# ThatRedox/ChunkyClPlugin

Hardware: NVIDIA B200
Metric: path samples/sec (higher is better)
Workload: dtype f32

## Files before the change

### chunkyclplugin_b200/csrc/ccu_layout.h

```cpp
#pragma once
#include <algorithm>
#include <cmath>
#include <cstdint>
#include <cstdlib>
#include <cstring>
#include <thread>
#include <unordered_map>
#include <vector>

#include "ccu_device.cuh"
#include "ccu_march.cuh"

namespace {
struct WideLayout {
    std::vector<unsigned> top, wide;
    int cell_level = 0, top_log2 = 0;
    bool ok = true;
};

inline unsigned wide_leaf(int word, int level, bool &ok) {
    long long v = -(long long)word;
    unsigned val;
    if (v == 0x7FFFFFFELL) val = CCU_WIDE_ANY;
    else if (v >= 0 && v < (long long)CCU_WIDE_ANY) val = (unsigned)v;
    else { ok = false; val = 0; }
    return CCU_WIDE_LEAF | ((unsigned)level << 26) | val;
}

unsigned wide_node(const int *tree, size_t n, int word, int lvl, WideLayout &b) {
    if (lvl < 2 || (size_t)word + 7 >= n) { b.ok = false; return wide_leaf(0, 0, b.ok); }
    const size_t idx = b.wide.size() / 64;
    if (idx >= 0x7FFFFFFFu) { b.ok = false; return wide_leaf(0, 0, b.ok); }
    b.wide.resize(b.wide.size() + 64);
    for (int i = 0; i < 4; i++)
        for (int j = 0; j < 4; j++)
            for (int k = 0; k < 4; k++) {
                unsigned e;
                int c1 = tree[(size_t)word + ((((i >> 1) & 1) << 2) | (((j >> 1) & 1) << 1) | ((k >> 1) & 1))];
                if (c1 <= 0) {
                    e = wide_leaf(c1, lvl - 1, b.ok);
                } else if ((size_t)c1 + 7 >= n) {
                    b.ok = false;
                    e = wide_leaf(0, 0, b.ok);
                } else {
                    int c2 = tree[(size_t)c1 + (((i & 1) << 2) | ((j & 1) << 1) | (k & 1))];
                    e = c2 <= 0 ? wide_leaf(c2, lvl - 2, b.ok) : wide_node(tree, n, c2, lvl - 2, b);
                }
                b.wide[idx * 64 + ((i << 4) | (j << 2) | k)] = e;
            }
    return (unsigned)idx;
}

struct AirLayout {
    std::vector<unsigned> top, wide, bricks;
    std::vector<unsigned char> wide_level;
    int cell_level = 4, top_log2 = 0;
    bool ok = true;
};

inline int layout_threads(int dim) {
    if (dim < 8) return 1;
    if (const char *e = getenv("CCU_COMMIT_THREADS")) return std::max(1, std::min(dim, atoi(e)));
    const unsigned hw = std::thread::hardware_concurrency();
    return (int)std::max(1u, std::min({hw ? hw : 4u, (unsigned)dim, 16u}));
}

inline unsigned air_leaf(int word, int level) { return CCU_WIDE_LEAF | ((word == 0 ? (unsigned)level : 31u) << 26); }
inline int oct_child(int x, int y, int z) { return ((x & 1) << 2) | ((y & 1) << 1) | (z & 1); }

unsigned air_brick(const int *tree, size_t n, int word, AirLayout &b) {
    const size_t idx = b.bricks.size() / 256;
    if (idx >= 0x7FFFFFu || (size_t)word + 7 >= n) { b.ok = false; return air_leaf(1, 0); }
    b.bricks.resize(b.bricks.size() + 256, 0u);
    for (int i = 0; i < 4; i++)
        for (int j = 0; j < 4; j++)
            for (int k = 0; k < 4; k++) {
                unsigned *blk = &b.bricks[idx * 256 + (size_t)((i << 4) | (j << 2) | k) * 4];
                unsigned uniform = 0;
                bool mixed = false;
                int c2 = 0;
                const int c1 = tree[(size_t)word + oct_child(i >> 1, j >> 1, k >> 1)];
                if (c1 <= 0) {
                    uniform = c1 == 0 ? (CCU_BRICK_UNIFORM | 3u) : 0u;
                } else if ((size_t)c1 + 7 >= n) {
                    b.ok = false;
                } else {
                    c2 = tree[(size_t)c1 + oct_child(i, j, k)];
                    if (c2 <= 0) uniform = c2 == 0 ? (CCU_BRICK_UNIFORM | 2u) : 0u;
                    else if ((size_t)c2 + 7 >= n) b.ok = false;
                    else mixed = true;
                }
                if (!mixed) {
                    blk[0] = blk[1] = blk[2] = blk[3] = uniform;
                    continue;
                }
                for (int x = 0; x < 4; x++)
                    for (int y = 0; y < 4; y++)
                        for (int z = 0; z < 4; z++) {
                            unsigned code;
                            const int d1 = tree[(size_t)c2 + oct_child(x >> 1, y >> 1, z >> 1)];
                            if (d1 <= 0) {
                                code = d1 == 0 ? 2u : 0u;
                            } else if ((size_t)d1 + 7 >= n) {
                                b.ok = false;
                                code = 0;
                            } else {
                                const int d2 = tree[(size_t)d1 + oct_child(x, y, z)];
                                if (d2 > 0) b.ok = false;
                                code = d2 == 0 ? 1u : 0u;
                            }
                            blk[x] |= code << ((((y << 2) | z)) * 2);
                        }
            }
    return (unsigned)idx;
}

unsigned air_node(const int *tree, size_t n, int word, int lvl, AirLayout &b) {
    if (lvl == 4) return air_brick(tree, n, word, b);
    if (lvl < 6 || (size_t)word + 7 >= n) { b.ok = false; return air_leaf(1, 0); }
    const size_t idx = b.wide.size() / 64;
    if (idx >= 0x1FFFFFFu) { b.ok = false; return air_leaf(1, 0); }
    b.wide.resize(b.wide.size() + 64);
    b.wide_level.push_back((unsigned char)lvl);
    for (int i = 0; i < 4; i++)
        for (int j = 0; j < 4; j++)
            for (int k = 0; k < 4; k++) {
                unsigned e;
                const int c1 = tree[(size_t)word + oct_child(i >> 1, j >> 1, k >> 1)];
                if (c1 <= 0) {
                    e = air_leaf(c1, lvl - 1);
                } else if ((size_t)c1 + 7 >= n) {
                    b.ok = false;
                    e = air_leaf(1, 0);
                } else {
                    const int c2 = tree[(size_t)c1 + oct_child(i, j, k)];
                    e = c2 <= 0 ? air_leaf(c2, lvl - 2) : air_node(tree, n, c2, lvl - 2, b);
                }
                b.wide[idx * 64 + ((i << 4) | (j << 2) | k)] = e;
            }
    return (unsigned)idx;
}

void air_small_brick(const int *tree, size_t n, int depth, AirLayout &b) {
    b.bricks.assign(256, 0u);
    const int size = 1 << depth;
    for (int x = 0; x < size; x++)
        for (int y = 0; y < size; y++)
            for (int z = 0; z < size; z++) {
                int level = depth, word = tree[0];
                while (word > 0 && level > 0) {
                    level--;
                    const size_t at = (size_t)word + oct_child(x >> level, y >> level, z >> level);
                    if (at >= n) { b.ok = false; word = -1; break; }
                    word = tree[at];
                }
                if (word > 0) { b.ok = false; word = -1; }
                unsigned *blk = &b.bricks[(size_t)((((x >> 2) & 3) << 4) | (((y >> 2) & 3) << 2) | ((z >> 2) & 3)) * 4];
                if (word == 0 && level >= 2) {
                    blk[x & 3] = CCU_BRICK_UNIFORM | (unsigned)level;
                } else {
                    const unsigned code = word == 0 ? (unsigned)level + 1u : 0u;
                    blk[x & 3] |= code << (((((y & 3) << 2) | (z & 3))) * 2);
                }
            }
}

inline void air_fill_slab(const int *tree, size_t n, int depth, int cl, int dim, int x0, int x1, unsigned *top, AirLayout &b) {
    for (int x = x0; x < x1 && b.ok; x++)
        for (int y = 0; y < dim; y++)
            for (int z = 0; z < dim; z++) {
                int level = depth;
                int word = tree[0];
                while (word > 0 && level > cl) {
                    level--;
                    const int sh = level - cl;
                    const size_t at = (size_t)word + oct_child(x >> sh, y >> sh, z >> sh);
                    if (at >= n) { b.ok = false; word = 0; break; }
                    word = tree[at];
                }
                top[((size_t)x * dim + y) * dim + z] = word <= 0 ? air_leaf(word, level) : air_node(tree, n, word, cl, b);
            }
}

AirLayout build_air_layout(const int *tree, size_t n, int depth) {
    AirLayout b;
    if (depth < 4) {
        b.cell_level = 4;
        b.top_log2 = 0;
        if (tree[0] <= 0) b.top.assign(1, air_leaf(tree[0], depth));
        else { b.top.assign(1, 0u); air_small_brick(tree, n, depth, b); }
    } else {
        int cl = std::max(depth - 7, 4);
        if (cl & 1) cl++;
        if (cl > depth) cl = depth & ~1;
        b.cell_level = cl;
        b.top_log2 = depth - cl;
        const int dim = 1 << b.top_log2;
        b.top.assign((size_t)dim * dim * dim, 0u);
        const int nt = layout_threads(dim);
        if (nt == 1) {
            air_fill_slab(tree, n, depth, cl, dim, 0, dim, b.top.data(), b);
        } else {
            std::vector<AirLayout> part(nt);
            std::vector<std::thread> th;
            for (int t = 0; t < nt; t++)
                th.emplace_back([&, t] { air_fill_slab(tree, n, depth, cl, dim, dim * t / nt, dim * (t + 1) / nt, b.top.data(), part[t]); });
            for (auto &t : th) t.join();
            for (int t = 0; t < nt; t++) {
                const unsigned wide_off = (unsigned)(b.wide.size() / 64), brick_off = (unsigned)(b.bricks.size() / 256);
                AirLayout &p = part[t];
                b.ok = b.ok && p.ok;
                for (size_t j = 0; j < p.wide_level.size(); j++) {
                    const unsigned off = p.wide_level[j] - 2 == 4 ? brick_off : wide_off;
                    for (int e = 0; e < 64; e++)
                        if (!(p.wide[j * 64 + e] & CCU_WIDE_LEAF)) p.wide[j * 64 + e] += off;
                }
                const unsigned top_off = cl == 4 ? brick_off : wide_off;
                const size_t c0 = (size_t)(dim * t / nt) * dim * dim, c1 = (size_t)(dim * (t + 1) / nt) * dim * dim;
                for (size_t c = c0; c < c1; c++)
                    if (!(b.top[c] & CCU_WIDE_LEAF)) b.top[c] += top_off;
                b.wide.insert(b.wide.end(), p.wide.begin(), p.wide.end());
                b.wide_level.insert(b.wide_level.end(), p.wide_level.begin(), p.wide_level.end());
                b.bricks.insert(b.bricks.end(), p.bricks.begin(), p.bricks.end());
            }
            if (b.wide.size() / 64 >= 0x1FFFFFFu || b.bricks.size() / 256 >= 0x7FFFFFu) b.ok = false;
        }
    }
    if (b.wide.empty()) b.wide.assign(64, air_leaf(1, 0));
    if (b.bricks.empty()) b.bricks.assign(256, 0u);
    return b;
}

struct BvhLayout {
    std::vector<int> rec;
    int root = 0;
    bool ok = true;
};
struct BvhStage {
    BvhLayout world, actor;
    std::vector<int> tris;
    std::unordered_map<int, int> leaf_at;
    bool ok = true;
    int leaf(const std::vector<int> &trigs, int prim, bool &valid) {
        auto [at, fresh] = leaf_at.try_emplace(prim, 0);
        if (!fresh) return at->second;
        if (prim < 0 || (size_t)prim >= trigs.size()) { valid = false; return 0; }
        const int count = trigs[(size_t)prim];
        if (count < 0 || (size_t)prim + 1 + (size_t)count * 20 > trigs.size()) { valid = false; return 0; }
        at->second = (int)(tris.size() / 8);
        tris.push_back(count);
        tris.insert(tris.end(), 7, 0);
        for (int i = 0; i < count; i++) {
            tris.insert(tris.end(), trigs.begin() + prim + 1 + (size_t)i * 20, trigs.begin() + prim + 1 + (size_t)(i + 1) * 20);
            tris.insert(tris.end(), 4, 0);
        }
        return at->second;
    }
};

int bvh_ref(const std::vector<int> &bvh, const std::vector<int> &trigs, size_t node, int depth, BvhLayout &b, BvhStage &s) {
    if (!b.ok) return -1;
    if (node + 6 >= bvh.size() || depth >= 64) { b.ok = false; return -1; }
    const int head = bvh[node];
    if (head <= 0) return -(1 + s.leaf(trigs, -head, b.ok));
    const size_t left = node + 7, right = (size_t)head;
    if (left + 6 >= bvh.size() || right + 6 >= bvh.size()) { b.ok = false; return -1; }
    const size_t r = b.rec.size() / 16;
    b.rec.resize(b.rec.size() + 16, 0);
    for (int i = 0; i < 6; i++) {
        b.rec[r * 16 + i] = bvh[left + 1 + i];
        b.rec[r * 16 + 8 + i] = bvh[right + 1 + i];
    }
    const int rl = bvh_ref(bvh, trigs, left, depth + 1, b, s);
    const int rr = bvh_ref(bvh, trigs, right, depth + 1, b, s);
    b.rec[r * 16 + 6] = rl;
    b.rec[r * 16 + 14] = rr;
    return (int)r;
}

inline bool bvh_is_empty(const std::vector<int> &bvh) {
    if (bvh.size() < 7) return true;
    if (bvh[0] != 0) return false;
// ... 322 lines not shown
```

### chunkyclplugin_b200/csrc/ccu_march.cuh

```cuda
#pragma once
#include "ccu_device.cuh"

namespace ccu {

#define CCU_BRICK_UNIFORM 0xC0000000u

struct LeanRay {
    float3 o, d, inv, doff;
    float t, limit;
    int steps;
    int fmx, fmy, fmz;
    float nmx, nmy, nmz;
};

__device__ __forceinline__ void lean_prepare(LeanRay &r) {
    r.doff = r.d * CCU_OFFSET;
    r.fmx = r.inv.x < 0.0f ? 0 : -1;
    r.fmy = r.inv.y < 0.0f ? 0 : -1;
    r.fmz = r.inv.z < 0.0f ? 0 : -1;
    r.nmx = r.inv.x < 0.0f ? -inff_() : nanf_();
    r.nmy = r.inv.y < 0.0f ? -inff_() : nanf_();
    r.nmz = r.inv.z < 0.0f ? -inff_() : nanf_();
}

__device__ __forceinline__ float lean_exit_axis(int b, int low, int fm, float q, float inv, float nm) {
    const int plane = ((b & ~low) | (low & fm)) - fm;
    return fmaxf(((float)plane - q) * inv, nm);
}

template <bool DEEP, bool TOPS>
__device__ __forceinline__ int lean_probe(const DScene &s, const unsigned *__restrict__ top, LeanRay &r) {
    if (r.steps >= s.draw_depth || r.t > r.limit) return 2;
    const float3 pos = r.o + r.d * r.t;
    const float3 q = pos + r.doff;
    const int bx = f2i(floorf(q.x)), by = f2i(floorf(q.y)), bz = f2i(floorf(q.z));
    if (((bx | by | bz) >> s.depth) != 0) return 2;
    const int tl = s.air_top_log2;
    unsigned e;
    if (!DEEP) {
        const unsigned ti = ((((unsigned)(bx >> 4) << tl) + (unsigned)(by >> 4)) << tl) + (unsigned)(bz >> 4);
        e = TOPS ? top[ti] : __ldg(top + ti);
    } else {
        int lvl = s.air_cell_level;
        const unsigned ti = ((((unsigned)(bx >> lvl) << tl) + (unsigned)(by >> lvl)) << tl) + (unsigned)(bz >> lvl);
        e = __ldg(top + ti);
        while (lvl > 4 && !(e & CCU_WIDE_LEAF)) {
            lvl -= 2;
            e = __ldg(s.air_wide + (e * 64u + (unsigned)((((bx >> lvl) & 3) << 4) | (((by >> lvl) & 3) << 2) | ((bz >> lvl) & 3))));
        }
    }
    int level;
    if (e & CCU_WIDE_LEAF) {
        level = ((int)(e << 1)) >> 27;
    } else {
        const unsigned wi = (unsigned)(((bx & 12) << 4) | ((by & 12) << 2) | (bz & 12) | (bx & 3));
        const unsigned w = __ldg(s.air_bricks + (e * 256u + wi));
        const int code = (int)((w >> ((((by & 3) << 2) | (bz & 3)) * 2)) & 3u);
        level = w >= CCU_BRICK_UNIFORM ? (int)(w & 31u) : code - 1;
    }
    if (level < 0) return 1;
    const int low = (1 << level) - 1;
    const float ex = lean_exit_axis(bx, low, r.fmx, q.x, r.inv.x, r.nmx);
    const float ey = lean_exit_axis(by, low, r.fmy, q.y, r.inv.y, r.nmy);
    const float ez = lean_exit_axis(bz, low, r.fmz, q.z, r.inv.z, r.nmz);
    r.t += fminf(ex, fminf(ey, ez)) + CCU_OFFSET;
    r.steps++;
    return 0;
}

template <bool TOPS>
__device__ __forceinline__ int lean_step_flat(const DScene &s, const unsigned *__restrict__ top, LeanRay &r, bool active, int done) {
    const bool fin0 = r.steps >= s.draw_depth || r.t > r.limit;
    const float3 pos = r.o + r.d * r.t;
    const float3 q = pos + r.doff;
    const int bx = f2i(floorf(q.x)), by = f2i(floorf(q.y)), bz = f2i(floorf(q.z));
    const bool fin = fin0 || (((bx | by | bz) >> s.depth) != 0);
    const int tl = s.air_top_log2;
    const unsigned ti = (((((unsigned)(bx >> 4) << tl) + (unsigned)(by >> 4)) << tl) + (unsigned)(bz >> 4)) & ((1u << (3 * tl)) - 1u);
    const unsigned e = TOPS ? top[ti] : __ldg(top + ti);
    const bool leaf = (e & CCU_WIDE_LEAF) != 0;
    const unsigned wi = (unsigned)(((bx & 12) << 4) | ((by & 12) << 2) | (bz & 12) | (bx & 3));
    const unsigned w = __ldg(s.air_bricks + (leaf ? 0u : e * 256u + wi));
    const int code = (int)((w >> ((((by & 3) << 2) | (bz & 3)) * 2)) & 3u);
    const int lvl_brick = w >= CCU_BRICK_UNIFORM ? (int)(w & 31u) : code - 1;
    const int level = leaf ? ((int)(e << 1)) >> 27 : lvl_brick;
    const int low = (1 << (level & 31)) - 1;
    const float ex = lean_exit_axis(bx, low, r.fmx, q.x, r.inv.x, r.nmx);
    const float ey = lean_exit_axis(by, low, r.fmy, q.y, r.inv.y, r.nmy);
    const float ez = lean_exit_axis(bz, low, r.fmz, q.z, r.inv.z, r.nmz);
    const float tn = r.t + (fminf(ex, fminf(ey, ez)) + CCU_OFFSET);
    const bool adv = active && !fin && level >= 0;
    r.t = adv ? tn : r.t;
    r.steps += adv ? 1 : 0;
    return active ? (fin ? 2 : (level < 0 ? 1 : 0)) : done;
}

template <bool DEEP, bool SPEC, bool CUT = false, bool BIOME = false>
__device__ __forceinline__ bool octree_intersect_lean(const DScene &s, float3 origin, float3 direction, RecordT<SPEC> &rec, HitInfo &hi) {
    March m;
    if (!march_begin(s, m, origin, direction, rec.distance)) return false;
    LeanRay r;
    r.o = m.o; r.d = m.d; r.inv = m.inv; r.t = m.t; r.limit = m.limit; r.steps = m.steps;
    lean_prepare(r);
    for (;;) {
        const int st = lean_probe<DEEP, false>(s, s.air_top, r);
        if (st == 0) continue;
        if (st == 2) return false;
        m.t = r.t; m.steps = r.steps;
        const Cell c = march_cell(m);
        int level;
        const int data = find_leaf_wide(s, c.bx, c.by, c.bz, level);
        float t;
        if (march_block<SPEC, CUT, BIOME>(s, m, data, level, rec.surf, t, CUT)) {
            rec.distance = t;
            rec.material = data;
            hi.node = -1;
            hi.kind = 1;
            hi.bx = c.bx; hi.by = c.by; hi.bz = c.bz;
            return true;
        }
        r.t = m.t; r.steps = m.steps;
    }
}

template <bool DEEP, bool SPEC, bool CUT = false, bool BIOME = false>
__device__ __forceinline__ bool closest_intersect_lean(const DScene &s, float3 origin, float3 direction, RecordT<SPEC> &rec, HitInfo &hi) {
    bool hit = octree_intersect_lean<DEEP, SPEC, CUT, BIOME>(s, origin, direction, rec, hi);
    int kind = 0;
    if (bvh_pair(s, origin, direction, rec.distance, rec.surf, kind)) {
        hit = true;
        hi.kind = kind;
        hi.node = -1;
    }
    if (hit) rec.point = origin + direction * (rec.distance - CCU_OFFSET);
    return hit;
}

template <int MODE, bool SPEC, bool CUT = false, bool BIOME = false>
__device__ __forceinline__ bool closest_intersect_mode(const DScene &s, float3 origin, float3 direction, RecordT<SPEC> &rec, HitInfo &hi) {
    if (MODE == 0) return closest_intersect_ref<SPEC, CUT, BIOME>(s, origin, direction, rec, hi);
    return closest_intersect_lean<MODE == 2, SPEC, CUT, BIOME>(s, origin, direction, rec, hi);
}

template <int MODE, bool SPEC, int NEE, bool BIOME>
__device__ __forceinline__ float3 sample_pixel(const DScene &s, const EmitView &g, int gid, int seed) {
    float3 color = f3(0, 0, 0), throughput = f3(1, 1, 1);
    int ray_depth = 0;
    uint32_t rng = (uint32_t)seed + (uint32_t)gid;
    rng_next(rng);
    float3 origin, direction;
    camera_ray<false>(s, gid, rng, origin, direction);
    RecordT<SPEC> rec;
    rec.distance = inff_();
    rec.material = 0;
    rec.point = f3(0, 0, 0);
    rec.surf.normal = f3(0, 0, 0);
    rec.surf.color = make_float4(0, 0, 0, 0);
    rec.surf.emittance = 0;
// ... 78 lines not shown
```

### chunkyclplugin_b200/csrc/ccu_queue.cuh

```cuda
#pragma once
#include "ccu_march.cuh"

#ifndef CCU_Q_WARPS
#define CCU_Q_WARPS 28
#endif
#ifndef CCU_Q_ROWS
#define CCU_Q_ROWS 32
#endif

namespace ccu {

constexpr int Q_WARPS = CCU_Q_WARPS;
constexpr int Q_ROWS = CCU_Q_ROWS;
constexpr int Q_SLOTS = Q_ROWS * 32;
constexpr int Q_MW = (Q_ROWS + 31) / 32;
static_assert(Q_ROWS >= 1 && Q_ROWS <= 64, "at most two mask words per stage and column");

enum QStage : int { QS_MARCH = 0, QS_BLOCK, QS_EXIT, QS_END, QS_BVH, QS_SHADE, QS_LEAF, QS_COUNT_BVH };
constexpr int QS_COUNT = QS_BVH;

enum QField : int {
    QF_GID = 0, QF_META, QF_RNG, QF_COLX, QF_COLY, QF_COLZ, QF_THRX, QF_THRY, QF_THRZ,
    QF_SNX, QF_SNY, QF_SNZ, QF_SHW,
    QF_OX, QF_OY, QF_OZ, QF_DX, QF_DY, QF_DZ, QF_IX, QF_IY, QF_IZ, QF_T, QF_LIMIT, QF_STEPS,
// ... 81 lines not shown
            if (old & bit) return w * 32 + __ffs((int)bit) - 1;
            QSTAT_LANE(15, 1);
            m = old & ~bit;
        }
    }
    return -1;
}
__device__ __forceinline__ void q_push(unsigned *mask, int stage, int lane, int row) {
    q_mask_or(mask + (stage * Q_MW + (Q_MW > 1 ? row >> 5 : 0)) * 32 + lane, 1u << (row & 31));
}
__device__ __forceinline__ bool q_has_work(const unsigned *mask, int stage, int lane) {
    unsigned any = 0;
#pragma unroll
    for (int w = 0; w < Q_MW; w++) any |= *(reinterpret_cast<const volatile unsigned *>(mask) + (stage * Q_MW + w) * 32 + lane);
    return any != 0;
}

__device__ __forceinline__ int q_pop_batch(unsigned *mask, int stage, int lane, int min_lanes) {
    const int row = q_pop(mask, stage, lane);
    if (min_lanes > 1) {
        const int got = __popc(__ballot_sync(0xffffffffu, row >= 0));
        if (got < min_lanes) {
            if (row >= 0) q_push(mask, stage, lane, row);
            return -2;
        }
    }
    return row;
}

__device__ __forceinline__ void bvh_first_ref(const DScene &s, int &ref, int &phase) {
    ref = 0;
    if (!s.world_bvh_empty) { phase = 0; ref = s.world_root; }
    else if (!s.actor_bvh_empty) { phase = 1; ref = s.actor_root; }
    else phase = 2;
}
__device__ __forceinline__ void bvh_phase_done(const DScene &s, int &ref, int &phase) {
    if (phase == 0 && !s.actor_bvh_empty) { phase = 1; ref = s.actor_root; }
    else { phase = 2; ref = 0; }
}

#define QI(f) (*reinterpret_cast<int *>(&F[(f) * Q_SLOTS + slot]))
#define QU(f) (F[(f) * Q_SLOTS + slot])
#define QFL(f) (*reinterpret_cast<float *>(&F[(f) * Q_SLOTS + slot]))

__device__ __forceinline__ void q_store_ray(uint32_t *F, unsigned *mask, int lane, int row, const March &m, bool entered) {
    const int slot = row * 32 + lane;
    QFL(QF_OX) = m.o.x; QFL(QF_OY) = m.o.y; QFL(QF_OZ) = m.o.z;
    QFL(QF_DX) = m.d.x; QFL(QF_DY) = m.d.y; QFL(QF_DZ) = m.d.z;
    QFL(QF_IX) = m.inv.x; QFL(QF_IY) = m.inv.y; QFL(QF_IZ) = m.inv.z;
    QFL(QF_T) = m.t; QFL(QF_LIMIT) = m.limit; QI(QF_STEPS) = m.steps;
    q_push(mask, entered ? QS_MARCH : QS_EXIT, lane, row);
}

__device__ __forceinline__ void q_load_lean(const uint32_t *F, int slot, LeanRay &r) {
    r.o = f3(__uint_as_float(F[QF_OX * Q_SLOTS + slot]), __uint_as_float(F[QF_OY * Q_SLOTS + slot]), __uint_as_float(F[QF_OZ * Q_SLOTS + slot]));
    r.d = f3(__uint_as_float(F[QF_DX * Q_SLOTS + slot]), __uint_as_float(F[QF_DY * Q_SLOTS + slot]), __uint_as_float(F[QF_DZ * Q_SLOTS + slot]));
    r.inv = f3(__uint_as_float(F[QF_IX * Q_SLOTS + slot]), __uint_as_float(F[QF_IY * Q_SLOTS + slot]), __uint_as_float(F[QF_IZ * Q_SLOTS + slot]));
    r.t = __uint_as_float(F[QF_T * Q_SLOTS + slot]);
    r.limit = __uint_as_float(F[QF_LIMIT * Q_SLOTS + slot]);
    r.steps = (int)F[QF_STEPS * Q_SLOTS + slot];
    lean_prepare(r);
}

template <int NST, int LAY>
__device__ __forceinline__ void q_stage_march(const DScene &s, const unsigned *__restrict__ top, uint32_t *F, unsigned *mask, int lane,
                                              int yield_below, int refill_min) {
    const unsigned full = 0xffffffffu;
    int cur = -1;
    LeanRay r;
    r.o = r.d = r.inv = r.doff = f3(0, 0, 0);
    r.t = 0; r.limit = 0; r.steps = 0; r.fmx = r.fmy = r.fmz = 0; r.nmx = r.nmy = r.nmz = 0;
    int done = 0;
    int recheck = 0;
    int busy = 0;
    int n_fly = 0;
    for (;;) {
        {
            if (cur < 0 || done != 0) {
                if (cur >= 0) {
                    F[QF_T * Q_SLOTS + cur] = __float_as_uint(r.t);
                    F[QF_STEPS * Q_SLOTS + cur] = (uint32_t)r.steps;
                    q_push(mask, done == 1 ? QS_BLOCK : QS_EXIT, cur & 31, cur >> 5);
                    done = 0;
                }
                const int row = q_pop(mask, QS_MARCH, lane);
                cur = row < 0 ? -1 : row * 32 + lane;
                if (cur >= 0) q_load_lean(F, cur, r);
            }
            busy = __popc(__ballot_sync(full, cur >= 0));
            QSTAT(24, 1);
            if (busy == 0) return;
            if (busy < yield_below) {
                if (recheck == 0) {
                    int best = 0;
#pragma unroll
                    for (int st = QS_BLOCK; st < NST; st++) best = max(best, __popc(__ballot_sync(full, q_has_work(mask, st, lane))));
                    if (best > busy) { QSTAT(13, 1); break; }
                    recheck = 4;
                }
                recheck--;
            }
        }
        do {
            if (LAY != 2) done = lean_step_flat<LAY == 0>(s, top, r, cur >= 0 && done == 0, done);
            else if (cur >= 0 && done == 0) done = lean_probe<LAY == 2, LAY == 0>(s, top, r);
            n_fly = __popc(__ballot_sync(full, cur >= 0 && done == 0));
            QSTAT(10, 1); QSTAT(11, n_fly);
        } while (busy - n_fly < refill_min && n_fly != 0);
    }
    if (cur >= 0) {
        F[QF_T * Q_SLOTS + cur] = __float_as_uint(r.t);
        F[QF_STEPS * Q_SLOTS + cur] = (uint32_t)r.steps;
        q_push(mask, done == 0 ? QS_MARCH : (done == 1 ? QS_BLOCK : QS_EXIT), cur & 31, cur >> 5);
    }
}

template <bool SPEC, int NEE, int NFI, bool BIOME>
__device__ __forceinline__ void q_shade(const DScene &s, const EmitView &g, uint32_t *F, unsigned *mask, int lane, int row, float3 o,
                                        float3 d, float distance, bool ray_hit, const SurfT<SPEC> &hit, bool covered) {
    const int slot = row * 32 + lane;
    uint32_t meta = QU(QF_META) & ~(NEE ? (QM_HIT | QM_COVERED) : QM_HIT);
    const bool shadow = (meta & QM_SHADOW) != 0;
    const bool nee_ray = NEE && (meta & QM_NEE_RAY) != 0;
    bool sun = false, bounce = false;
    bool nee_step = false;
    bool nee_ran = false;
    float3 from = o;
    float3 normal = f3(0, 0, 0);
    bool specular = false;
    float ro = 0;
    if (!ray_hit) {
        if (NEE && nee_ray) {
            float3 color = f3(QFL(QF_COLX), QFL(QF_COLY), QFL(QF_COLZ));
            color = color + f3(QFL(QF_SHW), QFL(NFI), QFL(NFI + 1));
            QFL(QF_COLX) = color.x; QFL(QF_COLY) = color.y; QFL(QF_COLZ) = color.z;
            bounce = true;
            nee_ran = true;
        } else {
            float3 throughput = f3(QFL(QF_THRX), QFL(QF_THRY), QFL(QF_THRZ));
            float3 color = f3(QFL(QF_COLX), QFL(QF_COLY), QFL(QF_COLZ));
            float3 sky = sky_radiance(s, d);
            color = color + (sky * throughput) * (shadow ? QFL(QF_SHW) : 1.0f);
            QFL(QF_COLX) = color.x; QFL(QF_COLY) = color.y; QFL(QF_COLZ) = color.z;
            if (shadow) { if (NEE) nee_step = true; else bounce = true; }
            else q_push(mask, QS_END, lane, row);
        }
    } else if (shadow) {
        if (NEE) nee_step = true; else bounce = true;
    } else if (NEE && nee_ray) {
        bounce = true;
        nee_ran = true;
    } else if (!SPEC) {
        float3 throughput = f3(QFL(QF_THRX), QFL(QF_THRY), QFL(QF_THRZ));
        float3 color = f3(QFL(QF_COLX), QFL(QF_COLY), QFL(QF_COLZ));
        from = o + d * (distance - CCU_OFFSET);
        float3 col = f3(hit.color.x, hit.color.y, hit.color.z);
        throughput = throughput * col;
        if (!(NEE && covered)) color = color + (col * (hit.emittance * s.emitter_scale)) * throughput;
        QFL(QF_THRX) = throughput.x; QFL(QF_THRY) = throughput.y; QFL(QF_THRZ) = throughput.z;
        QFL(QF_COLX) = color.x; QFL(QF_COLY) = color.y; QFL(QF_COLZ) = color.z;
        normal = hit.normal;
        if (s.sun_flags & 1) sun = true;
        else if (NEE) nee_step = true;
        else bounce = true;
    } else {
// ... 449 lines not shown
        }
        base1 = __shfl_sync(full, base1, leader);
        base2 = __shfl_sync(full, base2, leader);
        n1 = __shfl_sync(full, n1, leader);
        if (need_pixel) {
            const int rank = __popc(want & ((1u << lane) - 1u));
            const unsigned k = rank < n1 ? base1 + (unsigned)rank : base2 + (unsigned)(rank - n1);
            if (k < (unsigned)w.n_pixels) {
                gid = tile_order_pixel(LAST_FIRST ? (unsigned)w.n_pixels - 1u - k : k, s.width, s.height);
                pass = 0;
            } else {
                alive = false;
            }
        }
    }
    const unsigned died = __ballot_sync(full, row >= 0 && !alive);
    if (died && lane == (__ffs((int)died) - 1)) atomicSub(live, __popc(died));
    if (!alive) return true;
    QI(QF_GID) = gid;
    QU(QF_META) = (uint32_t)pass;
    QFL(QF_COLX) = 0.0f; QFL(QF_COLY) = 0.0f; QFL(QF_COLZ) = 0.0f;
    QFL(QF_THRX) = 1.0f; QFL(QF_THRY) = 1.0f; QFL(QF_THRZ) = 1.0f;
    uint32_t rng = (uint32_t)__ldg(w.seeds + pass) + (uint32_t)gid;
    rng_next(rng);
    float3 o, d;
    camera_ray<false>(s, gid, rng, o, d);
    QU(QF_RNG) = rng;
    March m;
    const bool entered = march_begin(s, m, o, d, inff_());
    q_store_ray(F, mask, lane, row, m, entered);
    return true;
}

template <bool HAS_BVH, int LAY, bool SPEC, int NEE, bool BIOME>
__global__ void __launch_bounds__(Q_WARPS * 32, 1) k_render_queue(const __grid_constant__ DScene s, const __grid_constant__ QueueParams qp,
                                                                 const __grid_constant__ EmitView g, const __grid_constant__ BiomeView bv) {
    constexpr int NST = q_stages(HAS_BVH);
    constexpr int MASK_WORDS = q_mask_words(HAS_BVH);
    extern __shared__ uint32_t q_mem[];
    uint32_t *F = q_mem;
    unsigned *mask = q_mem + q_fields(HAS_BVH, SPEC, NEE) * Q_SLOTS;
    int *live = reinterpret_cast<int *>(mask + MASK_WORDS);
    unsigned *top_s = mask + MASK_WORDS + 32;
    int *stk = reinterpret_cast<int *>(top_s + (LAY == 0 ? Q_TOP_WORDS : 0));
    const unsigned full = 0xffffffffu;
    const int lane = threadIdx.x & 31;

    for (int i = threadIdx.x; i < Q_SLOTS; i += blockDim.x) F[QF_META * Q_SLOTS + i] = QM_NEEDPIX;
    for (int i = threadIdx.x; i < NST * Q_MW * 32; i += blockDim.x) {
        const int st = i / (Q_MW * 32), w = (i / 32) % Q_MW;
        const int rows_here = min(32, Q_ROWS - 32 * w);
        mask[i] = st == QS_END ? (rows_here >= 32 ? 0xffffffffu : ((1u << rows_here) - 1u)) : 0u;
    }
    if (LAY == 0) {
        const int n = 1 << (3 * s.air_top_log2);
        for (int i = threadIdx.x; i < n; i += blockDim.x) top_s[i] = __ldg(s.air_top + i);
    }
    uchar4 *sky_s = nullptr;
    if (qp.sky_texels > 0) {
        sky_s = reinterpret_cast<uchar4 *>(top_s + (LAY == 0 ? Q_TOP_WORDS : 0) + (HAS_BVH ? Q_STACK_WORDS : 0));
        for (int i = threadIdx.x; i < qp.sky_texels; i += blockDim.x) sky_s[i] = __ldg(s.sky + i);
    }
    if constexpr (BIOME) {
        if (threadIdx.x == 0) biome_smem() = bv;
    }
    stage_tables(s, sky_s);
    if (threadIdx.x == 0) {
        live[0] = Q_SLOTS;
        live[1] = 0;
        live[2] = 0;
        live[3] = (int)Q_CHUNK;
    }
    __syncthreads();
    const unsigned *top = LAY == 0 ? top_s : s.air_top;

    int held = 0;
    int sticky = -1;
    for (;;) {
        int best = -1, best_n = 0;
        if (sticky >= 0) {
            int n = __popc(__ballot_sync(full, q_has_work(mask, sticky, lane)));
            int st2 = sticky;
            if (sticky == QS_BLOCK || sticky == QS_EXIT) {
                const int other = sticky == QS_BLOCK ? QS_EXIT : QS_BLOCK;
                const int n2 = __popc(__ballot_sync(full, q_has_work(mask, other, lane)));
                if (n2 > n) { n = n2; st2 = other; }
            }
            if (n >= qp.sticky_min) { best = st2; best_n = n; }
        }
        if (best < 0) {
#pragma unroll
        for (int st = 0; st < NST; st++) {
            int n = __popc(__ballot_sync(full, q_has_work(mask, st, lane)));
            if (st == QS_MARCH && n > 0) n = max(1, n + ((threadIdx.x >> 5 & 3) == 3 ? -qp.march_bias : qp.march_bias));
            if (st == QS_MARCH && (int)(threadIdx.x >> 5) >= qp.march_warps) n = 0;
            if (n > best_n) { best_n = n; best = st; }
        }
        }
        if (best < 0) {
            if (*reinterpret_cast<volatile int *>(live) == 0) break;
            QSTAT(12, 1);
            __nanosleep(100);
            continue;
        }
        const int min_lanes = held < 2 ? qp.shade_min : 1;
        bool ran = true;
        switch (best) {
            case QS_MARCH: QSTAT(0, 1); q_stage_march<NST, LAY>(s, top, F, mask, lane, qp.yield_below, qp.refill_min); break;
            case QS_BLOCK:
            case QS_EXIT: ran = q_stage_resolve<HAS_BVH, SPEC, NEE, BIOME>(s, g, F, mask, lane, best == QS_BLOCK, min_lanes); break;
// ... 22 lines not shown
```

### chunkyclplugin_b200/csrc/chunkycu.cu

```cuda
#include <cuda_runtime.h>

#include <algorithm>
#include <cmath>
#include <cstdarg>
#include <cstdio>
#include <cstdlib>
#include <cstring>
#include <climits>
#include <mutex>
#include <new>
#include <string>
#include <thread>
#include <vector>

#include <chrono>

#include "ccu_host.h"
#include "ccu_march.cuh"
#include "ccu_queue.cuh"
#include "ccu_tonemap.cuh"
#include "ccu_layout.h"

using namespace ccu;

// ... 20 lines not shown
    }
    stage_tables(s, nullptr);
    for (int gid = blockIdx.x * blockDim.x + threadIdx.x; gid < n_pixels; gid += gridDim.x * blockDim.x) {
        float *px = res + (size_t)gid * 3;
        const float *pp = res_prev + (size_t)gid * 3;
        float3 buf = f3(pp[0], pp[1], pp[2]);
        for (int pass = 0; pass < n_passes; pass++) {
            float3 col = sample_pixel<MODE, SPEC, NEE, BIOME>(s, g, gid, __ldg(seeds + pass));
            int spp = start_spp + pass;
            float fs = (float)spp, fs1 = (float)(spp + 1);
            buf.x = (buf.x * fs + col.x) / fs1;
            buf.y = (buf.y * fs + col.y) / fs1;
            buf.z = (buf.z * fs + col.z) / fs1;
        }
        px[0] = buf.x; px[1] = buf.y; px[2] = buf.z;
    }
}

__device__ __forceinline__ int face_of(float3 n) {
    if (n.x == -1 && n.y == 0 && n.z == 0) return 0;
    if (n.x == 1 && n.y == 0 && n.z == 0) return 1;
    if (n.x == 0 && n.y == -1 && n.z == 0) return 2;
    if (n.x == 0 && n.y == 1 && n.z == 0) return 3;
    if (n.x == 0 && n.y == 0 && n.z == -1) return 4;
    if (n.x == 0 && n.y == 0 && n.z == 1) return 5;
    return 6;
}

#ifndef CCU_FH_THREADS
#define CCU_FH_THREADS 128
#endif
#ifndef CCU_FH_MIN_BLOCKS
#define CCU_FH_MIN_BLOCKS (1024 / CCU_FH_THREADS)
#endif
struct FirstHitOut { int *block, *face, *node, *kind; float *t, *normal, *color; };
__device__ __forceinline__ void first_hit_store(const FirstHitOut &out, int gid, bool hit, int material, float3 n, int node, int kind, float t, float4 color) {
    if (out.block) out.block[gid] = hit ? material : 0;
    if (out.face) out.face[gid] = hit ? face_of(n) : 6;
    if (out.node) out.node[gid] = hit ? node : -1;
    if (out.kind) out.kind[gid] = hit ? kind : 0;
    if (out.t) out.t[gid] = hit ? t : inff_();
    if (out.normal) {
        out.normal[gid * 3 + 0] = hit ? n.x : 0.0f;
        out.normal[gid * 3 + 1] = hit ? n.y : 0.0f;
        out.normal[gid * 3 + 2] = hit ? n.z : 0.0f;
    }
    if (out.color) reinterpret_cast<float4 *>(out.color)[gid] = hit ? color : make_float4(0, 0, 0, 0);
}

template <bool DEEP>
static __device__ __noinline__ int first_hit_march(const DScene &s, LeanRay *ray, int st) {
    LeanRay r = *ray;
    while (__any_sync(0xffffffffu, st == 0)) {
        if (!DEEP) st = lean_step_flat<false>(s, s.air_top, r, st == 0, st);
        else if (st == 0) st = lean_probe<DEEP, false>(s, s.air_top, r);
    }
    ray->t = r.t;
    ray->steps = r.steps;
    return st;
}

template <int MODE, bool HAS_BVH>
__global__ void __launch_bounds__(CCU_FH_THREADS, CCU_FH_MIN_BLOCKS) k_first_hit(const __grid_constant__ DScene s, int seed, int n_pixels, const __grid_constant__ FirstHitOut out) {
    stage_tables_per_warp(s);
    const unsigned full = 0xffffffffu;
    const unsigned k = blockIdx.x * blockDim.x + threadIdx.x;
    const bool valid = k < (unsigned)n_pixels;
    unsigned px = 0, py = 0;
    if (valid) tile_order_xy<true>(k, s.width, s.height, px, py);
    const int gid = (int)(py * (unsigned)s.width + px);
    uint32_t rng = (uint32_t)seed + (uint32_t)gid;
    rng_next(rng);
    float3 o, d;
    camera_ray_xy<false>(s, gid, (int)px, (int)py, rng, o, d);
    if (MODE == 0) {
        Record rec;
        rec.distance = inff_(); rec.material = 0; rec.surf.normal = f3(0, 0, 0); rec.point = f3(0, 0, 0);
        rec.surf.color = make_float4(0, 0, 0, 0); rec.surf.emittance = 0;
        HitInfo hi = {-1, 0, 0, 0, 0};
        bool hit = false;
        if (valid) hit = HAS_BVH ? closest_intersect_ref(s, o, d, rec, hi) : octree_intersect_ref(s, o, d, rec, hi);
        if (valid) first_hit_store(out, gid, hit, rec.material, rec.surf.normal, hi.node, hi.kind, rec.distance, rec.surf.color);
        return;
    }
    March m;
    const bool entered = march_begin(s, m, o, d, inff_());
    LeanRay r;
    r.o = m.o; r.d = m.d; r.inv = m.inv; r.t = m.t; r.limit = m.limit; r.steps = m.steps;
    lean_prepare(r);
    int st = (valid && entered) ? 0 : 2;
    Surf surf;
    surf.normal = f3(0, 0, 0); surf.color = make_float4(0, 0, 0, 0); surf.emittance = 0;
    float distance = inff_();
    int material = 0, hbx = 0, hby = 0, hbz = 0;
    for (;;) {
        st = first_hit_march<MODE == 2>(s, &r, st);
        if (st == 1) {
            m.t = r.t; m.steps = r.steps;
            const Cell c = march_cell(m);
            int level;
            const int data = find_leaf_wide(s, c.bx, c.by, c.bz, level);
            float th;
            Surf hs;
            if (march_block(s, m, data, level, hs, th)) {
                st = 3;
                if (!HAS_BVH) {
                    int hnode = -1;
                    if (out.node) { int lv; find_leaf(s, c.bx, c.by, c.bz, lv, hnode); }
// ... 1353 lines not shown
    int rc;
    try {
        rc = check_biome_colors(chunks, rgb, n, "ccu_debug_biome_layout");
    } catch (const std::bad_alloc &) {
        return fail(CCU_ENOMEM, "ccu_debug_biome_layout: no host memory for %lld chunks", (long long)n);
    }
    if (rc != CCU_OK) return rc;
    BiomeLayout bl;
    rc = biome_layout(chunks, rgb, n, depth, bl, "ccu_debug_biome_layout");
    if (rc != CCU_OK) return rc;
    info[0] = bl.x0; info[1] = bl.z0; info[2] = bl.gx; info[3] = bl.gz;
    info[4] = (int)n;
    if (grid) std::copy(bl.grid.begin(), bl.grid.end(), grid);
    if (tiles) std::copy(bl.tiles.begin(), bl.tiles.end(), tiles);
    return CCU_OK;
}

int ccu_debug_layout_lookup(const int32_t *tree, int64_t n, int32_t depth, const int32_t *xyz, int64_t count, int32_t *wide_value,
                            int32_t *wide_level, int32_t *air_solid, int32_t *air_level) {
    if (!tree || n < 1 || depth < 0 || depth > 30 || (count > 0 && !xyz)) return fail(CCU_EINVAL, "ccu_debug_layout_lookup: bad argument");
    WideLayout wl = build_wide_layout(tree, (size_t)n, depth);
    AirLayout al = build_air_layout(tree, (size_t)n, depth);
    if (!al.ok) return fail(CCU_ESTATE, "air layout could not be built");
    const int cl = wl.cell_level, tl = wl.top_log2;
    for (int64_t i = 0; i < count; i++) {
        const int bx = xyz[3 * i], by = xyz[3 * i + 1], bz = xyz[3 * i + 2];
        if (((bx | by | bz) >> depth) != 0) return fail(CCU_EINVAL, "voxel %lld outside the octree cube", (long long)i);
        if (wl.ok) {
            const size_t cell = ((((size_t)(bx >> cl) << tl) + (size_t)(by >> cl)) << tl) + (size_t)(bz >> cl);
            unsigned e = wl.top[cell];
            int lvl = cl;
            while (!(e & CCU_WIDE_LEAF)) {
                lvl -= 2;
                e = wl.wide[(size_t)e * 64 + ((((bx >> lvl) & 3) << 4) | (((by >> lvl) & 3) << 2) | ((bz >> lvl) & 3))];
            }
            const unsigned v = e & CCU_WIDE_ANY;
            if (wide_value) wide_value[i] = v == CCU_WIDE_ANY ? CCU_ANY_TYPE : (int)v;
            if (wide_level) wide_level[i] = (int)((e >> 26) & 31);
        } else {
            if (wide_value) wide_value[i] = -1;
            if (wide_level) wide_level[i] = -1;
        }
        int lvl = al.cell_level;
        const int atl = al.top_log2;
        unsigned e = al.top[((((size_t)(bx >> lvl) << atl) + (size_t)(by >> lvl)) << atl) + (size_t)(bz >> lvl)];
        while (lvl > 4 && !(e & CCU_WIDE_LEAF)) {
            lvl -= 2;
            e = al.wide[(size_t)e * 64 + ((((bx >> lvl) & 3) << 4) | (((by >> lvl) & 3) << 2) | ((bz >> lvl) & 3))];
        }
        int level;
        if (e & CCU_WIDE_LEAF) {
            level = ((int)(e << 1)) >> 27;
        } else {
            const unsigned wi = (unsigned)(((bx & 12) << 4) | ((by & 12) << 2) | (bz & 12) | (bx & 3));
            const unsigned w = al.bricks[(size_t)e * 256 + wi];
            const int code = (int)((w >> ((((by & 3) << 2) | (bz & 3)) * 2)) & 3u);
            level = w >= CCU_BRICK_UNIFORM ? (int)(w & 31u) : code - 1;
        }
        if (air_solid) air_solid[i] = level < 0 ? 1 : 0;
        if (air_level) air_level[i] = level;
    }
    return CCU_OK;
}

}
```

Before: 3.152 billion.

## Store per-voxel 4-bit air levels in 16³ bricks, drop leaf branches in march

Replaces the 2-bit/uniform-flag brick encoding with a 4-bit per-voxel empty-level nibble layout (512 words per brick). Top-level leaves now point at shared constant bricks, so the flat march no longer branches on leaf vs brick. The top grid is padded to 16³ for a shift-only index. Draw-depth is folded into the step counter and the refill loop condition is simplified, removing a few per-step comparisons. In exchange bricks use twice the memory, and all per-voxel entries inside a brick are now filled with finer empty-level data.

```diff
diff --git a/chunkyclplugin_b200/csrc/ccu_layout.h b/chunkyclplugin_b200/csrc/ccu_layout.h
--- a/chunkyclplugin_b200/csrc/ccu_layout.h
+++ b/chunkyclplugin_b200/csrc/ccu_layout.h
@@ -58,6 +58,8 @@
     bool ok = true;
 };
 
+constexpr size_t AIR_MAX_BRICKS = 0x400000;
+
 inline int layout_threads(int dim) {
     if (dim < 8) return 1;
     if (const char *e = getenv("CCU_COMMIT_THREADS")) return std::max(1, std::min(dim, atoi(e)));
@@ -68,51 +70,37 @@
 inline unsigned air_leaf(int word, int level) { return CCU_WIDE_LEAF | ((word == 0 ? (unsigned)level : 31u) << 26); }
 inline int oct_child(int x, int y, int z) { return ((x & 1) << 2) | ((y & 1) << 1) | (z & 1); }
 
+inline unsigned air_code(int word, int level) { return word == 0 ? (unsigned)level : (unsigned)CCU_AIR_SOLID; }
+inline void air_brick_set(unsigned *brick, int x, int y, int z, unsigned code) {
+    brick[ccu::air_brick_word(x, y, z)] |= code << ((z & 7) * 4);
+}
+
 unsigned air_brick(const int *tree, size_t n, int word, AirLayout &b) {
-    const size_t idx = b.bricks.size() / 256;
-    if (idx >= 0x7FFFFFu || (size_t)word + 7 >= n) { b.ok = false; return air_leaf(1, 0); }
-    b.bricks.resize(b.bricks.size() + 256, 0u);
-    for (int i = 0; i < 4; i++)
-        for (int j = 0; j < 4; j++)
-            for (int k = 0; k < 4; k++) {
-                unsigned *blk = &b.bricks[idx * 256 + (size_t)((i << 4) | (j << 2) | k) * 4];
-                unsigned uniform = 0;
-                bool mixed = false;
-                int c2 = 0;
-                const int c1 = tree[(size_t)word + oct_child(i >> 1, j >> 1, k >> 1)];
-                if (c1 <= 0) {
-                    uniform = c1 == 0 ? (CCU_BRICK_UNIFORM | 3u) : 0u;
-                } else if ((size_t)c1 + 7 >= n) {
-                    b.ok = false;
-                } else {
-                    c2 = tree[(size_t)c1 + oct_child(i, j, k)];
-                    if (c2 <= 0) uniform = c2 == 0 ? (CCU_BRICK_UNIFORM | 2u) : 0u;
-                    else if ((size_t)c2 + 7 >= n) b.ok = false;
-                    else mixed = true;
+    const size_t idx = b.bricks.size() / CCU_BRICK_WORDS;
+    if (idx >= AIR_MAX_BRICKS || (size_t)word + 7 >= n) { b.ok = false; return air_leaf(1, 0); }
+    b.bricks.resize(b.bricks.size() + CCU_BRICK_WORDS, 0u);
+    unsigned *brick = &b.bricks[idx * CCU_BRICK_WORDS];
+    for (int x = 0; x < 16; x++)
+        for (int y = 0; y < 16; y++)
+            for (int z = 0; z < 16; z++) {
+                int level = 4, w = word;
+                while (w > 0 && level > 0) {
+                    if ((size_t)w + 7 >= n) { b.ok = false; w = -1; break; }
+                    level--;
+                    w = tree[(size_t)w + oct_child(x >> level, y >> level, z >> level)];
                 }
-                if (!mixed) {
-                    blk[0] = blk[1] = blk[2] = blk[3] = uniform;
-                    continue;
-                }
-                for (int x = 0; x < 4; x++)
-                    for (int y = 0; y < 4; y++)
-                        for (int z = 0; z < 4; z++) {
-                            unsigned code;
-                            const int d1 = tree[(size_t)c2 + oct_child(x >> 1, y >> 1, z >> 1)];
-                            if (d1 <= 0) {
-                                code = d1 == 0 ? 2u : 0u;
-                            } else if ((size_t)d1 + 7 >= n) {
-                                b.ok = false;
-                                code = 0;
-                            } else {
-                                const int d2 = tree[(size_t)d1 + oct_child(x, y, z)];
-                                if (d2 > 0) b.ok = false;
-                                code = d2 == 0 ? 1u : 0u;
-                            }
-                            blk[x] |= code << ((((y << 2) | z)) * 2);
-                        }
-            }
-    return (unsigned)idx;
+                if (w > 0) { b.ok = false; w = -1; }
+                air_brick_set(brick, x, y, z, air_code(w, level));
+            }
+    return (unsigned)(idx * CCU_BRICK_WORDS);
+}
+
+unsigned air_const_brick(AirLayout &b, std::vector<unsigned> &made, unsigned code) {
+    if (made[code] == ~0u) {
+        made[code] = (unsigned)b.bricks.size();
+        b.bricks.resize(b.bricks.size() + CCU_BRICK_WORDS, code * 0x11111111u);
+    }
+    return made[code];
 }
 
 unsigned air_node(const int *tree, size_t n, int word, int lvl, AirLayout &b) {
@@ -142,12 +130,13 @@
 }
 
 void air_small_brick(const int *tree, size_t n, int depth, AirLayout &b) {
-    b.bricks.assign(256, 0u);
+    b.bricks.assign(CCU_BRICK_WORDS, 0u);
     const int size = 1 << depth;
-    for (int x = 0; x < size; x++)
-        for (int y = 0; y < size; y++)
-            for (int z = 0; z < size; z++) {
+    for (int x = 0; x < 16; x++)
+        for (int y = 0; y < 16; y++)
+            for (int z = 0; z < 16; z++) {
                 int level = depth, word = tree[0];
+                if (x >= size || y >= size || z >= size) word = -1;
                 while (word > 0 && level > 0) {
                     level--;
                     const size_t at = (size_t)word + oct_child(x >> level, y >> level, z >> level);
@@ -155,13 +144,7 @@
                     word = tree[at];
                 }
                 if (word > 0) { b.ok = false; word = -1; }
-                unsigned *blk = &b.bricks[(size_t)((((x >> 2) & 3) << 4) | (((y >> 2) & 3) << 2) | ((z >> 2) & 3)) * 4];
-                if (word == 0 && level >= 2) {
-                    blk[x & 3] = CCU_BRICK_UNIFORM | (unsigned)level;
-                } else {
-                    const unsigned code = word == 0 ? (unsigned)level + 1u : 0u;
-                    blk[x & 3] |= code << (((((y & 3) << 2) | (z & 3))) * 2);
-                }
+                air_brick_set(b.bricks.data(), x, y, z, air_code(word, level));
             }
 }
 
@@ -207,15 +190,15 @@
                 th.emplace_back([&, t] { air_fill_slab(tree, n, depth, cl, dim, dim * t / nt, dim * (t + 1) / nt, b.top.data(), part[t]); });
             for (auto &t : th) t.join();
             for (int t = 0; t < nt; t++) {
-                const unsigned wide_off = (unsigned)(b.wide.size() / 64), brick_off = (unsigned)(b.bricks.size() / 256);
+                const unsigned wide_off = (unsigned)(b.wide.size() / 64), brick_off = (unsigned)(b.bricks.size() / CCU_BRICK_WORDS);
                 AirLayout &p = part[t];
                 b.ok = b.ok && p.ok;
                 for (size_t j = 0; j < p.wide_level.size(); j++) {
-                    const unsigned off = p.wide_level[j] - 2 == 4 ? brick_off : wide_off;
+                    const unsigned off = p.wide_level[j] - 2 == 4 ? brick_off * CCU_BRICK_WORDS : wide_off;
                     for (int e = 0; e < 64; e++)
                         if (!(p.wide[j * 64 + e] & CCU_WIDE_LEAF)) p.wide[j * 64 + e] += off;
                 }
-                const unsigned top_off = cl == 4 ? brick_off : wide_off;
+                const unsigned top_off = cl == 4 ? brick_off * CCU_BRICK_WORDS : wide_off;
                 const size_t c0 = (size_t)(dim * t / nt) * dim * dim, c1 = (size_t)(dim * (t + 1) / nt) * dim * dim;
                 for (size_t c = c0; c < c1; c++)
                     if (!(b.top[c] & CCU_WIDE_LEAF)) b.top[c] += top_off;
@@ -223,11 +206,29 @@
                 b.wide_level.insert(b.wide_level.end(), p.wide_level.begin(), p.wide_level.end());
                 b.bricks.insert(b.bricks.end(), p.bricks.begin(), p.bricks.end());
             }
-            if (b.wide.size() / 64 >= 0x1FFFFFFu || b.bricks.size() / 256 >= 0x7FFFFFu) b.ok = false;
-        }
+            if (b.wide.size() / 64 >= 0x1FFFFFFu || b.bricks.size() / CCU_BRICK_WORDS >= AIR_MAX_BRICKS) b.ok = false;
+        }
+    }
+    if (b.cell_level == 4 && b.top_log2 < 4) {
+        const int dim = 1 << b.top_log2;
+        std::vector<unsigned> t((size_t)16 * 16 * 16, air_leaf(1, 0));
+        for (int x = 0; x < dim; x++)
+            for (int y = 0; y < dim; y++)
+                for (int z = 0; z < dim; z++) t[(size_t)((x << 8) | (y << 4) | z)] = b.top[((size_t)x * dim + y) * dim + z];
+        b.top.swap(t);
+        b.top_log2 = 4;
+    }
+    if (b.cell_level == 4) {
+        std::vector<unsigned> made(16, ~0u);
+        for (unsigned &e : b.top)
+            if (e & CCU_WIDE_LEAF) {
+                const unsigned level = (e >> 26) & 31u;
+                e = air_const_brick(b, made, level == 31 ? (unsigned)CCU_AIR_SOLID : level);
+            }
+        if (b.bricks.size() / CCU_BRICK_WORDS >= AIR_MAX_BRICKS) b.ok = false;
     }
     if (b.wide.empty()) b.wide.assign(64, air_leaf(1, 0));
-    if (b.bricks.empty()) b.bricks.assign(256, 0u);
+    if (b.bricks.empty()) b.bricks.assign(CCU_BRICK_WORDS, CCU_AIR_SOLID * 0x11111111u);
     return b;
 }
 
diff --git a/chunkyclplugin_b200/csrc/ccu_march.cuh b/chunkyclplugin_b200/csrc/ccu_march.cuh
--- a/chunkyclplugin_b200/csrc/ccu_march.cuh
+++ b/chunkyclplugin_b200/csrc/ccu_march.cuh
@@ -3,7 +3,19 @@
 
 namespace ccu {
 
-#define CCU_BRICK_UNIFORM 0xC0000000u
+#define CCU_BRICK_WORDS 512u
+#define CCU_AIR_SOLID 15
+
+__host__ __device__ __forceinline__ unsigned air_brick_word(int x, int y, int z) {
+    return (((unsigned)x & 15u) << 5) | (((unsigned)y & 15u) << 1) | (((unsigned)z >> 3) & 1u);
+}
+__host__ __device__ __forceinline__ int air_brick_level(unsigned w, int z) {
+#ifdef __CUDA_ARCH__
+    return (int)(__funnelshift_r(w, w, (unsigned)z << 2) & 15u);
+#else
+    return (int)((w >> ((z & 7) * 4)) & 15u);
+#endif
+}
 
 struct LeanRay {
     float3 o, d, inv, doff;
@@ -29,8 +41,8 @@
 }
 
 template <bool DEEP, bool TOPS>
-__device__ __forceinline__ int lean_probe(const DScene &s, const unsigned *__restrict__ top, LeanRay &r) {
-    if (r.steps >= s.draw_depth || r.t > r.limit) return 2;
+__device__ __forceinline__ int lean_probe(const DScene &s, const unsigned *__restrict__ top, LeanRay &r, int draw_depth) {
+    if (r.steps >= draw_depth || r.t > r.limit) return 2;
     const float3 pos = r.o + r.d * r.t;
     const float3 q = pos + r.doff;
     const int bx = f2i(floorf(q.x)), by = f2i(floorf(q.y)), bz = f2i(floorf(q.z));
@@ -50,15 +62,13 @@
         }
     }
     int level;
-    if (e & CCU_WIDE_LEAF) {
-        level = ((int)(e << 1)) >> 27;
+    if (DEEP && (e & CCU_WIDE_LEAF)) {
+        level = (int)((e >> 26) & 31u);
+        if (level == 31) return 1;
     } else {
-        const unsigned wi = (unsigned)(((bx & 12) << 4) | ((by & 12) << 2) | (bz & 12) | (bx & 3));
-        const unsigned w = __ldg(s.air_bricks + (e * 256u + wi));
-        const int code = (int)((w >> ((((by & 3) << 2) | (bz & 3)) * 2)) & 3u);
-        level = w >= CCU_BRICK_UNIFORM ? (int)(w & 31u) : code - 1;
-    }
-    if (level < 0) return 1;
+        level = air_brick_level(__ldg(s.air_bricks + (e + air_brick_word(bx, by, bz))), bz);
+        if (level == CCU_AIR_SOLID) return 1;
+    }
     const int low = (1 << level) - 1;
     const float ex = lean_exit_axis(bx, low, r.fmx, q.x, r.inv.x, r.nmx);
     const float ey = lean_exit_axis(by, low, r.fmy, q.y, r.inv.y, r.nmy);
@@ -68,31 +78,33 @@
     return 0;
 }
 
-template <bool TOPS>
-__device__ __forceinline__ int lean_step_flat(const DScene &s, const unsigned *__restrict__ top, LeanRay &r, bool active, int done) {
-    const bool fin0 = r.steps >= s.draw_depth || r.t > r.limit;
+template <bool TOP16>
+__device__ __forceinline__ int lean_step_flat(const DScene &s, const unsigned *__restrict__ top, LeanRay &r, bool active, int done,
+                                              int draw_depth, unsigned outside) {
+    const bool fin0 = r.steps >= draw_depth || r.t > r.limit;
     const float3 pos = r.o + r.d * r.t;
     const float3 q = pos + r.doff;
     const int bx = f2i(floorf(q.x)), by = f2i(floorf(q.y)), bz = f2i(floorf(q.z));
-    const bool fin = fin0 || (((bx | by | bz) >> s.depth) != 0);
-    const int tl = s.air_top_log2;
-    const unsigned ti = (((((unsigned)(bx >> 4) << tl) + (unsigned)(by >> 4)) << tl) + (unsigned)(bz >> 4)) & ((1u << (3 * tl)) - 1u);
-    const unsigned e = TOPS ? top[ti] : __ldg(top + ti);
-    const bool leaf = (e & CCU_WIDE_LEAF) != 0;
-    const unsigned wi = (unsigned)(((bx & 12) << 4) | ((by & 12) << 2) | (bz & 12) | (bx & 3));
-    const unsigned w = __ldg(s.air_bricks + (leaf ? 0u : e * 256u + wi));
-    const int code = (int)((w >> ((((by & 3) << 2) | (bz & 3)) * 2)) & 3u);
-    const int lvl_brick = w >= CCU_BRICK_UNIFORM ? (int)(w & 31u) : code - 1;
-    const int level = leaf ? ((int)(e << 1)) >> 27 : lvl_brick;
-    const int low = (1 << (level & 31)) - 1;
+    const bool fin = fin0 || ((unsigned)(bx | by | bz) & outside) != 0;
+    unsigned ti;
+    if (TOP16) {
+        ti = (((unsigned)bx << 4) & 0xF00u) | ((unsigned)by & 0xF0u) | (((unsigned)bz >> 4) & 0xFu);
+    } else {
+        const int tl = s.air_top_log2;
+        ti = (((((unsigned)(bx >> 4) << tl) + (unsigned)(by >> 4)) << tl) + (unsigned)(bz >> 4)) & ((1u << (3 * tl)) - 1u);
+    }
+    const unsigned e = TOP16 ? top[ti] : __ldg(top + ti);
+    const int level = air_brick_level(__ldg(s.air_bricks + (e + air_brick_word(bx, by, bz))), bz);
+    const int low = (1 << level) - 1;
     const float ex = lean_exit_axis(bx, low, r.fmx, q.x, r.inv.x, r.nmx);
     const float ey = lean_exit_axis(by, low, r.fmy, q.y, r.inv.y, r.nmy);
     const float ez = lean_exit_axis(bz, low, r.fmz, q.z, r.inv.z, r.nmz);
     const float tn = r.t + (fminf(ex, fminf(ey, ez)) + CCU_OFFSET);
-    const bool adv = active && !fin && level >= 0;
+    const bool air = level != CCU_AIR_SOLID;
+    const bool adv = active && !fin && air;
     r.t = adv ? tn : r.t;
     r.steps += adv ? 1 : 0;
-    return active ? (fin ? 2 : (level < 0 ? 1 : 0)) : done;
+    return active ? (fin ? 2 : (air ? 0 : 1)) : done;
 }
 
 template <bool DEEP, bool SPEC, bool CUT = false, bool BIOME = false>
@@ -103,7 +115,7 @@
     r.o = m.o; r.d = m.d; r.inv = m.inv; r.t = m.t; r.limit = m.limit; r.steps = m.steps;
     lean_prepare(r);
     for (;;) {
-        const int st = lean_probe<DEEP, false>(s, s.air_top, r);
+        const int st = lean_probe<DEEP, false>(s, s.air_top, r, s.draw_depth);
         if (st == 0) continue;
         if (st == 2) return false;
         m.t = r.t; m.steps = r.steps;
diff --git a/chunkyclplugin_b200/csrc/ccu_queue.cuh b/chunkyclplugin_b200/csrc/ccu_queue.cuh
--- a/chunkyclplugin_b200/csrc/ccu_queue.cuh
+++ b/chunkyclplugin_b200/csrc/ccu_queue.cuh
@@ -157,40 +157,47 @@
     q_push(mask, entered ? QS_MARCH : QS_EXIT, lane, row);
 }
 
-__device__ __forceinline__ void q_load_lean(const uint32_t *F, int slot, LeanRay &r) {
+__device__ __forceinline__ void q_load_lean(const uint32_t *F, int slot, LeanRay &r, int draw_depth) {
     r.o = f3(__uint_as_float(F[QF_OX * Q_SLOTS + slot]), __uint_as_float(F[QF_OY * Q_SLOTS + slot]), __uint_as_float(F[QF_OZ * Q_SLOTS + slot]));
     r.d = f3(__uint_as_float(F[QF_DX * Q_SLOTS + slot]), __uint_as_float(F[QF_DY * Q_SLOTS + slot]), __uint_as_float(F[QF_DZ * Q_SLOTS + slot]));
     r.inv = f3(__uint_as_float(F[QF_IX * Q_SLOTS + slot]), __uint_as_float(F[QF_IY * Q_SLOTS + slot]), __uint_as_float(F[QF_IZ * Q_SLOTS + slot]));
     r.t = __uint_as_float(F[QF_T * Q_SLOTS + slot]);
     r.limit = __uint_as_float(F[QF_LIMIT * Q_SLOTS + slot]);
-    r.steps = (int)F[QF_STEPS * Q_SLOTS + slot];
+    r.steps = (int)F[QF_STEPS * Q_SLOTS + slot] - draw_depth;
     lean_prepare(r);
+}
+__device__ __forceinline__ void q_store_lean_t(uint32_t *F, int slot, const LeanRay &r, int draw_depth) {
+    F[QF_T * Q_SLOTS + slot] = __float_as_uint(r.t);
+    F[QF_STEPS * Q_SLOTS + slot] = (uint32_t)(r.steps + draw_depth);
 }
 
 template <int NST, int LAY>
 __device__ __forceinline__ void q_stage_march(const DScene &s, const unsigned *__restrict__ top, uint32_t *F, unsigned *mask, int lane,
                                               int yield_below, int refill_min) {
     const unsigned full = 0xffffffffu;
+    const int draw_depth = s.draw_depth;
+    const unsigned outside = ~0u << s.depth;
     int cur = -1;
     LeanRay r;
     r.o = r.d = r.inv = r.doff = f3(0, 0, 0);
     r.t = 0; r.limit = 0; r.steps = 0; r.fmx = r.fmy = r.fmz = 0; r.nmx = r.nmy = r.nmz = 0;
-    int done = 0;
+    int done = 2;
     int recheck = 0;
     int busy = 0;
     int n_fly = 0;
     for (;;) {
         {
-            if (cur < 0 || done != 0) {
+            if (done != 0) {
                 if (cur >= 0) {
-                    F[QF_T * Q_SLOTS + cur] = __float_as_uint(r.t);
-                    F[QF_STEPS * Q_SLOTS + cur] = (uint32_t)r.steps;
+                    q_store_lean_t(F, cur, r, draw_depth);
                     q_push(mask, done == 1 ? QS_BLOCK : QS_EXIT, cur & 31, cur >> 5);
-                    done = 0;
                 }
                 const int row = q_pop(mask, QS_MARCH, lane);
                 cur = row < 0 ? -1 : row * 32 + lane;
-                if (cur >= 0) q_load_lean(F, cur, r);
+                done = cur < 0 ? 2 : 0;
+                if (cur >= 0) q_load_lean(F, cur, r, draw_depth);
+                else r.steps = 0;
+
             }
             busy = __popc(__ballot_sync(full, cur >= 0));
             QSTAT(24, 1);
@@ -206,16 +213,16 @@
                 recheck--;
             }
         }
+        const int fly_min = max(busy - refill_min, 0);
         do {
-            if (LAY != 2) done = lean_step_flat<LAY == 0>(s, top, r, cur >= 0 && done == 0, done);
-            else if (cur >= 0 && done == 0) done = lean_probe<LAY == 2, LAY == 0>(s, top, r);
-            n_fly = __popc(__ballot_sync(full, cur >= 0 && done == 0));
+            if (LAY != 2) done = lean_step_flat<LAY == 0>(s, top, r, true, 0, 0, outside);
+            else if (done == 0) done = lean_probe<LAY == 2, LAY == 0>(s, top, r, 0);
+            n_fly = __popc(__ballot_sync(full, done == 0));
             QSTAT(10, 1); QSTAT(11, n_fly);
-        } while (busy - n_fly < refill_min && n_fly != 0);
+        } while (n_fly > fly_min);
     }
     if (cur >= 0) {
-        F[QF_T * Q_SLOTS + cur] = __float_as_uint(r.t);
-        F[QF_STEPS * Q_SLOTS + cur] = (uint32_t)r.steps;
+        q_store_lean_t(F, cur, r, draw_depth);
         q_push(mask, done == 0 ? QS_MARCH : (done == 1 ? QS_BLOCK : QS_EXIT), cur & 31, cur >> 5);
     }
 }
@@ -771,10 +778,7 @@
         const int rows_here = min(32, Q_ROWS - 32 * w);
         mask[i] = st == QS_END ? (rows_here >= 32 ? 0xffffffffu : ((1u << rows_here) - 1u)) : 0u;
     }
-    if (LAY == 0) {
-        const int n = 1 << (3 * s.air_top_log2);
-        for (int i = threadIdx.x; i < n; i += blockDim.x) top_s[i] = __ldg(s.air_top + i);
-    }
+    if (LAY == 0) for (int i = threadIdx.x; i < Q_TOP_WORDS; i += blockDim.x) top_s[i] = __ldg(s.air_top + i);
     uchar4 *sky_s = nullptr;
     if (qp.sky_texels > 0) {
         sky_s = reinterpret_cast<uchar4 *>(top_s + (LAY == 0 ? Q_TOP_WORDS : 0) + (HAS_BVH ? Q_STACK_WORDS : 0));
diff --git a/chunkyclplugin_b200/csrc/chunkycu.cu b/chunkyclplugin_b200/csrc/chunkycu.cu
--- a/chunkyclplugin_b200/csrc/chunkycu.cu
+++ b/chunkyclplugin_b200/csrc/chunkycu.cu
@@ -96,8 +96,8 @@
 static __device__ __noinline__ int first_hit_march(const DScene &s, LeanRay *ray, int st) {
     LeanRay r = *ray;
     while (__any_sync(0xffffffffu, st == 0)) {
-        if (!DEEP) st = lean_step_flat<false>(s, s.air_top, r, st == 0, st);
-        else if (st == 0) st = lean_probe<DEEP, false>(s, s.air_top, r);
+        if (!DEEP) st = lean_step_flat<false>(s, s.air_top, r, st == 0, st, s.draw_depth, ~0u << s.depth);
+        else if (st == 0) st = lean_probe<DEEP, false>(s, s.air_top, r, s.draw_depth);
     }
     ray->t = r.t;
     ray->steps = r.steps;
@@ -1557,10 +1557,8 @@
         if (e & CCU_WIDE_LEAF) {
             level = ((int)(e << 1)) >> 27;
         } else {
-            const unsigned wi = (unsigned)(((bx & 12) << 4) | ((by & 12) << 2) | (bz & 12) | (bx & 3));
-            const unsigned w = al.bricks[(size_t)e * 256 + wi];
-            const int code = (int)((w >> ((((by & 3) << 2) | (bz & 3)) * 2)) & 3u);
-            level = w >= CCU_BRICK_UNIFORM ? (int)(w & 31u) : code - 1;
+            const int code = air_brick_level(al.bricks[(size_t)e + air_brick_word(bx, by, bz)], bz);
+            level = code == CCU_AIR_SOLID ? -1 : code;
         }
         if (air_solid) air_solid[i] = level < 0 ? 1 : 0;
         if (air_level) air_level[i] = level;
```

Result: faster. 3.342 billion, median of 6 (+6.0%).
